# nsdumont/Semantic-Spiking-Neural-SLAM-2023

Measured on AMD Instinct MI355X. Metric: sim-sec/wall-sec, SSP-SLAM ssp_dim=1015 10k PI neurons, 1/2/4/8 MI355X, higher is better.
Workload: dtype f32; 1 GPU; PathIntegration 2-D ssp_dim=1015 pi_n_neurons=10000/VCO (508 VCOs, 5080000 LIF neurons), configs[1]; eval_points_per_vco=4000, parallelism=1 GPU, build_cache=miss

## Files before the change

semantic-spiking-neural-slam-2023_amd/csrc/ssn_block.hpp:

```cpp
#pragma once
#include <type_traits>
#include "ssn_launch.hpp"

namespace ssn {

__device__ inline float wave_sum_dpp(float v) {
  int x;
#define SSN_DPP_ADD(ctrl, rmask)                                                                             \
  x = __builtin_amdgcn_update_dpp(0, __builtin_bit_cast(int, v), ctrl, rmask, 0xF, false);                    \
  v += __builtin_bit_cast(float, x);
  SSN_DPP_ADD(0xB1, 0xF)
  SSN_DPP_ADD(0x4E, 0xF)
  SSN_DPP_ADD(0x141, 0xF)
  SSN_DPP_ADD(0x140, 0xF)
  SSN_DPP_ADD(0x142, 0xA)
  SSN_DPP_ADD(0x143, 0xC)
#undef SSN_DPP_ADD
  return v;
}
__device__ inline float row_sum_dpp(float v) {
  int x;
#define SSN_DPP_ADD(ctrl)                                                                                    \
  x = __builtin_amdgcn_update_dpp(0, __builtin_bit_cast(int, v), ctrl, 0xF, 0xF, false);                      \
  v += __builtin_bit_cast(float, x);
  SSN_DPP_ADD(0xB1) SSN_DPP_ADD(0x4E) SSN_DPP_ADD(0x141) SSN_DPP_ADD(0x140)
#undef SSN_DPP_ADD
  return v;
}
template <int N>
__device__ inline void wave_sum_dpp_n(float* v) {
#define SSN_DPP_STAGE(ctrl, rmask)                                                                            \
  _Pragma("unroll") for (int r = 0; r < N; ++r) {                                                              \
    const int x = __builtin_amdgcn_update_dpp(0, __builtin_bit_cast(int, v[r]), ctrl, rmask, 0xF, false);      \
    v[r] += __builtin_bit_cast(float, x);                                                                      \
  }
  SSN_DPP_STAGE(0xB1, 0xF) SSN_DPP_STAGE(0x4E, 0xF) SSN_DPP_STAGE(0x141, 0xF) SSN_DPP_STAGE(0x140, 0xF)
  SSN_DPP_STAGE(0x142, 0xA) SSN_DPP_STAGE(0x143, 0xC)
#undef SSN_DPP_STAGE
}
__device__ inline double wave_sum_dpp(double v) {
#pragma unroll
  for (int off = 32; off > 0; off >>= 1) v += __shfl_xor(v, off, 64);
  return v;
}
template <int N>
__device__ inline void wave_sum_dpp_n(double* v) {
#pragma unroll
  for (int r = 0; r < N; ++r) v[r] = wave_sum_dpp(v[r]);
}

typedef float f32x2 __attribute__((ext_vector_type(2)));
typedef unsigned int u32x2 __attribute__((ext_vector_type(2)));
__device__ inline f32x2 pk_clamp01(f32x2 x) {
  f32x2 r;
  asm("v_pk_mul_f32 %0, %1, 1.0 op_sel_hi:[1,0] clamp" : "=v"(r) : "v"(x));
  return r;
}
__device__ inline f32x2 pk_sub_clamp01(f32x2 x, f32x2 y) {
  f32x2 r;
  asm("v_pk_add_f32 %0, %1, %2 neg_lo:[0,1] neg_hi:[0,1] clamp" : "=v"(r) : "v"(x), "s"(y));
  return r;
}
__device__ inline f32x2 pk_mul_clamp01(f32x2 x, f32x2 y) {
  f32x2 r;
  asm("v_pk_mul_f32 %0, %1, %2 clamp" : "=v"(r) : "v"(x), "s"(y));
  return r;
}
__device__ inline f32x2 pk_fma_clamp01_vsv(f32x2 x, f32x2 y, f32x2 z) {
  f32x2 r;
  asm("v_pk_fma_f32 %0, %1, %2, %3 clamp" : "=v"(r) : "v"(x), "s"(y), "v"(z));
  return r;
}
__device__ inline f32x2 pk_fma_clamp01_trans_vvs(f32x2 x, f32x2 y, f32x2 z) {
  f32x2 r;
  asm("s_nop 0\n\tv_pk_fma_f32 %0, %1, %2, %3 clamp" : "=v"(r) : "v"(x), "v"(y), "s"(z));
  return r;
}

__device__ inline f32x2 pk_fma_clamp01_vs_negv(f32x2 x, f32x2 y, f32x2 z) {
  f32x2 r;
  asm("v_pk_fma_f32 %0, %1, %2, %3 neg_lo:[0,0,1] neg_hi:[0,0,1] clamp" : "=v"(r) : "v"(x), "s"(y), "v"(z));
  return r;
}

struct LifConstV3 { float na, ca, m1, c1, c2, c3, p0, p1, p2, ktau_ref, K; };
struct LifConstV3P { f32x2 na, ca, m1, c1, c2, c3, p0, p1, p2, ktau_ref; };

__device__ inline LifConstV3 lif_const_v3(double dt, double tau_rc, double tau_ref) {
  double K = 1.0;
  while (2.0 * K * tau_ref <= 1.0 && K < 1048576.0) K *= 2.0;
  while (K * tau_ref > 1.0) K *= 0.5;
  const double h = dt / tau_rc;
  const double x0 = h, x1 = 0.5 * h, x2 = 0.0669872981077807 * h;
  auto f = [](double x) { return -expm1(-x) / x; };
  const double f0 = f(x0), f1 = f(x1), f2 = f(x2);
  const double d01 = (f1 - f0) / (x1 - x0), d12 = (f2 - f1) / (x2 - x1), d012 = (d12 - d01) / (x2 - x0);
  const double q2 = d012, q1 = d01 - d012 * (x0 + x1), q0 = f0 - d01 * x0 + d012 * x0 * x1;
  LifConstV3 c;
  const float a = (float)(1.0 / (K * dt));
  float ca = a + 1.0f;
  if ((double)ca < (double)a + 1.0) ca = __builtin_bit_cast(float, __builtin_bit_cast(unsigned int, ca) + 1u);
  c.na = -a; c.ca = ca; c.m1 = (float)(1.0 + K * dt);
  c.c1 = (float)(q0 * h); c.c2 = (float)(q1 * h * h); c.c3 = (float)(q2 * h * h * h);
  {
    const double um = -expm1(-h);
    const double u0 = um * 0.9330127018922193, u1 = um * 0.5, u2 = um * 0.0669872981077807;
    auto phi = [](double u) { return log1p(-u) / u; };
    const double g0 = phi(u0), g1 = phi(u1), g2 = phi(u2);
    const double e01 = (g1 - g0) / (u1 - u0), e12 = (g2 - g1) / (u2 - u1), e012 = (e12 - e01) / (u2 - u0);
    const double r2 = e012, r1 = e01 - e012 * (u0 + u1), r0 = g0 - e01 * u0 + e012 * u0 * u1;
    c.p0 = (float)(K * tau_rc * r0); c.p1 = (float)(K * tau_rc * r1); c.p2 = (float)(K * tau_rc * r2);
  }
  c.ktau_ref = (float)(K * tau_ref); c.K = (float)K;
  return c;
}

__device__ inline f32x2 lif_state_dl(f32x2 w, f32x2 na, f32x2 ca) {
  return pk_fma_clamp01_vsv(w, (f32x2)(na), (f32x2)(ca));
}
__device__ inline f32x2 lif_state_p1(f32x2 dl, f32x2 c3, f32x2 c2) {
  f32x2 P;
  asm("v_pk_fma_f32 %0, %1, %2, %3" : "=v"(P) : "v"(dl), "v"((f32x2)(c3)), "s"((f32x2)(c2)));
  return P;
}
__device__ inline f32x2 lif_state_p2(f32x2 dl, f32x2 P, f32x2 c1) {
  asm("v_pk_fma_f32 %0, %1, %2, %3" : "=v"(P) : "v"(dl), "v"(P), "s"((f32x2)(c1)));
  return P;
}
__device__ inline void lif_state_part(f32x2 w, const LifConstV3P& c, f32x2& W0, f32x2& em) {
  W0 = pk_clamp01(w);
  const f32x2 dl = lif_state_dl(w, c.na, c.ca);
  const f32x2 P = lif_state_p2(dl, lif_state_p1(dl, c.c3, c.c2), c.c1);
  em = dl * P;
}
__device__ inline f32x2 lif_spike_test(f32x2 Jm1, f32x2 w, f32x2 W0, f32x2 em, const LifConstV3P& c, f32x2 big, f32x2& U, f32x2& nmt) {
  nmt = pk_sub_clamp01(w, (f32x2)(c.m1));
  U = __builtin_elementwise_fma(Jm1 + W0, em, -W0);
  return pk_mul_clamp01(U, big);
}
__device__ inline void lif_finish_spiking(f32x2 Jm1, f32x2& w, f32x2 U, f32x2 nmt, f32x2 spk, const LifConstV3P& c, f32x2 big) {
  f32x2 rc;
  rc.x = __builtin_amdgcn_rcpf(Jm1.x);
  rc.y = __builtin_amdgcn_rcpf(Jm1.y);
  const f32x2 u = U * rc;
  f32x2 P, nu;
  asm("v_pk_fma_f32 %0, %1, %2, %3" : "=v"(P) : "v"(u), "v"((f32x2)(c.p2)), "s"((f32x2)(c.p1)));
  asm("v_pk_fma_f32 %0, %1, %2, %3" : "=v"(P) : "v"(u), "v"(P), "s"((f32x2)(c.p0)));
  asm("v_pk_fma_f32 %0, %1, %2, %3 clamp" : "=v"(nu) : "v"(u), "v"(P), "s"((f32x2)(c.ktau_ref)));
  const f32x2 Wn = pk_fma_clamp01_vs_negv(spk, big, U);
  w = __builtin_elementwise_fma(spk, nu, Wn + nmt);
}
__device__ inline void lif_finish_silent(f32x2& w, f32x2 U, f32x2 nmt) {
  f32x2 Wn;
  asm("v_pk_mul_f32 %0, %1, -1.0 op_sel_hi:[1,0] clamp" : "=v"(Wn) : "v"(U));
  w = Wn + nmt;
}
__device__ inline f32x2 lif_input_part(f32x2 Jm1, f32x2& w, f32x2 W0, f32x2 em, const LifConstV3P& c, f32x2 big) {
  const f32x2 nmt = pk_sub_clamp01(w, (f32x2)(c.m1));
  const f32x2 U = __builtin_elementwise_fma(Jm1 + W0, em, -W0);
  const f32x2 spk = pk_mul_clamp01(U, big);
  f32x2 rc;
  rc.x = __builtin_amdgcn_rcpf(Jm1.x);
  rc.y = __builtin_amdgcn_rcpf(Jm1.y);
  f32x2 Wn, u, P, nu;
  asm("v_pk_fma_f32 %0, %2, %3, %4 neg_lo:[0,0,1] neg_hi:[0,0,1] clamp\n\t"
      "v_pk_mul_f32 %1, %4, %5"
      : "=&v"(Wn), "=v"(u)
      : "v"(spk), "s"(big), "v"(U), "v"(rc));
  asm("v_pk_fma_f32 %0, %1, %2, %3" : "=v"(P) : "v"(u), "v"((f32x2)(c.p2)), "s"((f32x2)(c.p1)));
  asm("v_pk_fma_f32 %0, %1, %2, %3" : "=v"(P) : "v"(u), "v"(P), "s"((f32x2)(c.p0)));
  asm("v_pk_fma_f32 %0, %1, %2, %3 clamp" : "=v"(nu) : "v"(u), "v"(P), "s"((f32x2)(c.ktau_ref)));
  w = __builtin_elementwise_fma(spk, nu, Wn + nmt);
  return spk;
}
__device__ inline float lif_word_in(float s, float K) { return __builtin_fmaf(-s, s < 0.0f ? K : 1.0f, 1.0f); }
__device__ inline float lif_word_out(float w, float K) { return (1.0f - w) * (w > 1.0f ? 1.0f / K : 1.0f); }

__device__ inline float bits_f(unsigned int x) { return __builtin_bit_cast(float, x); }
__device__ inline unsigned int f_bits(float x) { return __builtin_bit_cast(unsigned int, x); }

#ifdef SSN_BLOCK_STAMPS
__device__ unsigned long long g_block_stamps[9];
inline hipError_t read_block_stamps(unsigned long long* out, int reset) {
  hipError_t e = hipMemcpyFromSymbol(out, HIP_SYMBOL(g_block_stamps), sizeof(unsigned long long) * 9);
  if (e == hipSuccess && reset) {
    const unsigned long long z[9] = {0, 0, 0, 0, 0, 0, 0, 0, 0};
    e = hipMemcpyToSymbol(HIP_SYMBOL(g_block_stamps), z, sizeof z);
  }
  return e;
}
#define SSN_BSTAMP(var)                                                                          \
  do {                                                                                           \
    __builtin_amdgcn_sched_barrier(0);                                                           \
    asm volatile("s_memtime %0\n\ts_waitcnt lgkmcnt(0)" : "=s"(var) :: "memory");                \
    __builtin_amdgcn_sched_barrier(0);                                                           \
  } while (0)
#define SSN_BSTAMP_ADD(i, a, b) bst[i] += (b) - (a)
#else
#define SSN_BSTAMP(var) do {} while (0)
#define SSN_BSTAMP_ADD(i, a, b) do {} while (0)
#endif

#ifndef SSN_BLOCK_SKIP
#define SSN_BLOCK_SKIP 0
#endif
#ifndef SSN_BLOCK_PIPE
#define SSN_BLOCK_PIPE 1
#endif
#ifndef SSN_BLOCK_HOIST_A
#define SSN_BLOCK_HOIST_A 2
#endif
#ifndef SSN_BLOCK_HOIST_B
#define SSN_BLOCK_HOIST_B 4
#endif
#ifndef SSN_BLOCK_HOIST_C
#define SSN_BLOCK_HOIST_C 2
#endif
struct BlockHoist { int a, b, c; };
constexpr BlockHoist block_hoist(bool pipe, int tpb, int ng) {
  if (!pipe || SSN_BLOCK_SKIP != 0) return {0, 0, 0};
  const int room = tpb <= 512 && ng >= 10 ? ng : 0;
  const int c = SSN_BLOCK_HOIST_C >= 2 && room >= 2 ? 2 : 0;
  int b = SSN_BLOCK_HOIST_B < room - c ? SSN_BLOCK_HOIST_B : room - c;
  int a_ = SSN_BLOCK_HOIST_A < room - c - b ? SSN_BLOCK_HOIST_A : room - c - b;
  return {a_, b, c};
}

template <typename T, int DIN, int DOUT, int NPT, int TPB, int LDSW, int SPLIT = 0, int TAP = 0>
__global__ __launch_bounds__(TPB) void k_ens_block(BlockArgs<T> a) {
  static_assert(!(SPLIT && TAP), "the split kernel has no tapped form");
  constexpr bool ENC_LDS = LDSW == DIN;
  static_assert(LDSW == 0 || LDSW == DIN, "LDSW");
  extern __shared__ __align__(16) unsigned char ssn_block_dyn[];
  T* const e_lds = reinterpret_cast<T*>(ssn_block_dyn);
  constexpr bool F32 = sizeof(T) == 4;
  constexpr int PK = F32 ? 2 : 1;
  constexpr int NG = NPT / PK;
  static_assert(NPT % PK == 0, "f32 variants handle neuron pairs");
  constexpr bool PIPE = F32 && NG >= 5 && SSN_BLOCK_PIPE != 0;
  constexpr BlockHoist HO = block_hoist(PIPE, TPB, NG);
  constexpr int HC = HO.c, HA = HO.a, HB = HO.b, HT = HC + HA + HB;
  using G = typename std::conditional<F32, f32x2, T>::type;
  constexpr int DP = DOUT <= 4 ? 4 : 8;
  static_assert(!SPLIT || (sizeof(T) == 4 && DOUT <= 4), "split ensembles: f32, at most four decoded rows");
  const int P = SPLIT ? a.P : 1;
  const int k = P > 1 ? (int)blockIdx.x / P : (int)blockIdx.x;
  const int member = P > 1 ? (int)blockIdx.x - k * P : 0;
  const int noff = member * a.n_member;
  const int n_loc = P > 1 ? max(0, min(a.n_member, a.n_pad - noff)) : a.n_pad;
  const int tid = threadIdx.x;
  const int nthr = NG == 1 ? (int)blockDim.x : TPB;
  const int lane = tid & 63, wave = tid >> 6;
  const size_t row = (size_t)a.n_pad;
  const T* __restrict__ enc = a.enc + (size_t)k * DIN * row + noff;
  const T* __restrict__ bias = a.bias + (size_t)k * row + noff;
  T* __restrict__ Sp = a.S + (size_t)k * row + noff;
  const NeuronParams<T> np = a.np;
  const LifMath<T> lm(np);
  const int* tcol = nullptr;
  if constexpr (TAP != 0) {
    const int tslot = a.tap_slot[k];
    if (tslot >= 0) tcol = a.tap_col + (size_t)tslot * row;
  }
  auto uni = [](float v) { return bits_f(__builtin_amdgcn_readfirstlane(f_bits(v))); };
  const LifConstV3 lc0 = lif_const_v3((double)np.dt, (double)np.tau_rc, (double)np.tau_ref);
  auto uni2 = [&](float v) { const float u = uni(v); return (f32x2){u, u}; };
  const LifConstV3P lc = {uni2(lc0.na), uni2(lc0.ca), uni2(lc0.m1), uni2(lc0.c1), uni2(lc0.c2), uni2(lc0.c3), uni2(lc0.p0), uni2(lc0.p1),
                          uni2(lc0.p2), uni2(lc0.ktau_ref)};
  const float lcK = uni(lc0.K);
  const f32x2 big = {0x1p100f, 0x1p100f};

  G e[ENC_LDS ? 1 : NG][DIN], b[NG], s[NG], dc[NG][DOUT];
  constexpr int cap = (NG == 1 ? 1024 : TPB) * NPT;
  int lrow[LDSW > 0 ? LDSW : 1];
#pragma unroll
  for (int d = 0; d < (LDSW > 0 ? LDSW : 1); ++d) {
    lrow[d] = d * cap + tid * PK;
    asm volatile("" : "+v"(lrow[d]));
  }
  auto lds_group = [&](int d, int g) -> const G* {
    return reinterpret_cast<const G*>(e_lds + lrow[d] + g * nthr * PK);
  };
#pragma unroll
  for (int g = 0; g < NG; ++g) {
    const int i0 = (g * nthr + tid) * PK;
    const bool in = i0 < n_loc;
    const int ii = in ? i0 : 0;
    const T msk = in ? T(1) : T(0);
    auto ld = [&](const T* p) -> G { if constexpr (F32) return *reinterpret_cast<const f32x2*>(p) * msk; else return *p * msk; };
#pragma unroll
    for (int d = 0; d < DIN; ++d) {
      const G ev = ld(enc + d * row + ii);
      if constexpr (ENC_LDS) *reinterpret_cast<G*>(e_lds + d * cap + i0) = ev; else e[g][d] = ev;
    }
    b[g] = ld(bias + ii);
    s[g] = ld(Sp + ii);
    if constexpr (F32) {
      b[g] = b[g] - 1.0f;
      s[g] = (f32x2){lif_word_in(s[g].x, lcK), lif_word_in(s[g].y, lcK)};
    }
    if (a.dec_neuron_major) {
      const T* dp = a.dec + ((size_t)k * row + noff + ii) * DP;
#pragma unroll
      for (int r = 0; r < DOUT; ++r) {
        if constexpr (F32) dc[g][r] = (f32x2){dp[r], dp[DP + r]} * msk; else dc[g][r] = dp[r] * msk;
      }
    } else {
      const T* dp = a.dec + (size_t)k * DOUT * row + noff + ii;
#pragma unroll
      for (int r = 0; r < DOUT; ++r) dc[g][r] = ld(dp + r * row);
    }
  }

  constexpr int CH = 32;
  constexpr int XP = 4;
  constexpr int RW = DOUT <= 4 ? 64 : 128;
  __shared__ __align__(16) T red[2][RW];
  __shared__ __align__(16) T xs[CH][XP];
  __shared__ T os[CH][DOUT];
  __shared__ int s_dst[DOUT];
  __shared__ int s_out[DOUT];
  for (int i = tid; i < 2 * RW; i += nthr) (&red[0][0])[i] = T(0);
  if (tid < DOUT) { s_dst[tid] = a.didx[(long long)k * DOUT + tid]; s_out[tid] = a.rowout[(long long)k * DOUT + tid] ? 1 : 0; }
  const T* __restrict__ xbase = a.xrows + (size_t)a.row0 * a.n_sig + a.x_off + (long long)k * DIN;

  T fs[F32 ? 1 : DOUT], la[F32 ? 1 : DOUT], lb[F32 ? 1 : DOUT], tot[F32 ? 1 : DOUT];
  float F0 = 0.0f, F1 = 0.0f, la0 = 0.0f, lb0 = 0.0f, la1 = 0.0f, lb1 = 0.0f, v0 = 0.0f, v1 = 0.0f;
  T xa[DIN];
  int xr[DIN];
#pragma unroll
  for (int d = 0; d < DIN; ++d) {
    xr[d] = a.xrow[(long long)k * DIN + d];
    xa[d] = xr[d] >= 0 ? a.xalpha[(long long)k * DIN + d] : T(0);
  }
  if constexpr (F32) {
    const int r0 = lane >> 4;
    if (r0 < DOUT) {
      const long long i = (long long)k * DOUT + r0;
      const int st = a.lp_state[i];
      if (st >= 0) { F0 = a.sig[st]; la0 = a.lp_a[i]; lb0 = a.lp_b[i]; }
    }
    if (DOUT > 4) {
      const long long i = (long long)k * DOUT + 4;
      const int st = a.lp_state[i];
      if (st >= 0) { F1 = a.sig[st]; la1 = a.lp_a[i]; lb1 = a.lp_b[i]; }
    }
  } else {
#pragma unroll
    for (int r = 0; r < DOUT; ++r) {
      const long long i = (long long)k * DOUT + r;
      const int st = a.lp_state[i];
      fs[r] = st >= 0 ? a.sig[st] : T(0);
      la[r] = st >= 0 ? a.lp_a[i] : T(0);
      lb[r] = st >= 0 ? a.lp_b[i] : T(0);
      tot[r] = T(0);
    }
  }
  int wslot = -1;
  if constexpr (F32) {
    if constexpr (DOUT >= 4) {
      const int rv = (lane >> 4) == 1 ? 2 : ((lane >> 4) == 2 ? 1 : (lane >> 4));
      if ((lane & 15) == 0) wslot = rv * 16 + wave;
      if (DOUT == 5 && lane == 63) wslot = 64 + wave;
    }
  }

  constexpr int ILE = F32 ? (SSN_BLOCK_IL < NG ? SSN_BLOCK_IL : NG) : 1;
  G en[ILE][LDSW > 0 ? LDSW : 1];
  if constexpr (ENC_LDS) {
#pragma unroll
    for (int u = 0; u < ILE; ++u)
#pragma unroll
      for (int d = 0; d < LDSW; ++d) en[u][d] = *lds_group(d, u);
  }
#ifdef SSN_BLOCK_STAMPS
  unsigned long long bst[6] = {0, 0, 0, 0, 0, 0}, bt0 = 0, bt1 = 0, bt2 = 0, bt3 = 0, bt4 = 0, bt5 = 0, bt6 = 0, bm0 = 0, br0 = 0;
  asm volatile("s_memtime %0\n\ts_memrealtime %1\n\ts_waitcnt lgkmcnt(0)" : "=s"(bm0), "=s"(br0) :: "memory");
#endif
  unsigned int n_slots = 0, n_silent = 0;
  T x[DIN];
  int xl[DIN];
#pragma unroll
  for (int d = 0; d < DIN; ++d) xl[d] = __builtin_amdgcn_readfirstlane((xr[d] & 3) << 4);
  auto assemble_x = [&](const float4 xv) {
    const float xin[4] = {xv.x, xv.y, xv.z, xv.w};
    float f1 = 0.0f;
    if constexpr (DOUT > 4) f1 = bits_f(__builtin_amdgcn_readlane(f_bits(F1), 0));
#pragma unroll
    for (int d = 0; d < DIN; ++d) {
      const float f0 = bits_f(__builtin_amdgcn_readlane(f_bits(F0), xl[d]));
      float st = f0;
      if constexpr (DOUT > 4) st = xr[d] >= 4 ? f1 : f0;
      x[d] = __builtin_fmaf(xa[d], st, xin[d]);
    }
  };
  f32x2 W0h[HT > 0 ? HT : 1], emh[HT > 0 ? HT : 1];
  if constexpr (HT > 0) {
#pragma unroll
    for (int g = 0; g < HT; ++g) lif_state_part(s[g], lc, W0h[g], emh[g]);
  }
  for (int j0 = 0; j0 < a.B; j0 += CH) {
    const int cn = min(CH, a.B - j0);
    __syncthreads();
    if (j0 > 0 && member == 0) {
      for (int i = tid; i < CH * DOUT; i += nthr) {
        const int jj = i / DOUT, r = i - jj * DOUT;
        if (s_out[r]) a.bsig[(size_t)(a.row0 + j0 - CH + jj) * a.n_sig + s_dst[r]] = os[jj][r];
      }
    }
    for (int i = tid; i < cn * DIN; i += nthr) {
      const int jj = i / DIN, d = i - jj * DIN;
      xs[jj][d] = xbase[(size_t)(j0 + jj) * a.n_sig + d];
    }
    __syncthreads();
    if constexpr (PIPE) {
      assemble_x(*(const float4*)xs[0]);
    }

    for (int jj = 0; jj < cn; ++jj) {
      SSN_BSTAMP(bt0);
      if constexpr (SPLIT != 0) {
        if (P > 1 && wave == 0 && (lane & 15) == 0) {
          unsigned int* const rst = a.xslots + (size_t)k * 64 + (size_t)((j0 + jj + 1) % 3) * ((size_t)a.K * 64) + member * 4 + (lane >> 4);
          const unsigned int sent = BLOCK_XCHG_SENTINEL;
          asm volatile("global_store_dword %0, %1, off sc0 sc1" :: "v"(rst), "v"(sent) : "memory");
        }
      }
      if constexpr (PIPE) {
      } else if constexpr (F32) {
        assemble_x(*(const float4*)xs[jj]);
      } else {
        T xin[XP];
        *(double2*)xin = *(const double2*)xs[jj]; *(double2*)(xin + 2) = *(const double2*)(xs[jj] + 2);
#pragma unroll
        for (int d = 0; d < DIN; ++d) {
          T st = T(0);
#pragma unroll
          for (int r = 0; r < DOUT; ++r) st = xr[d] == r ? fs[r] : st;
          x[d] = xr[d] >= 0 ? xin[d] + xa[d] * st : xin[d];
        }
      }
      SSN_BSTAMP(bt1);
      G accg[DOUT];
#pragma unroll
      for (int r = 0; r < DOUT; ++r) accg[r] = G(0);
      constexpr int IL = ILE;
#pragma unroll
      for (int g0 = 0; g0 < NG; g0 += IL) {
        G J[IL], spk[IL];
#pragma unroll
        for (int u = 0; u < IL; ++u) {
          const int g = g0 + u < NG ? g0 + u : NG - 1;
          J[u] = b[g];
#pragma unroll
          for (int d = 0; d < DIN; ++d) {
            if constexpr (ENC_LDS) J[u] += en[u][d] * x[d];
            else J[u] += e[g][d] * x[d];
          }
        }
        if constexpr (ENC_LDS) {
#pragma unroll
          for (int u = 0; u < IL; ++u) {
            if (g0 + u >= NG) continue;
            asm volatile("" : "+v"(J[u]));
            const int gn = g0 + IL + u < NG ? g0 + IL + u : (g0 + IL + u) % IL;
#pragma unroll
            for (int d = 0; d < LDSW; ++d) en[u][d] = *lds_group(d, gn);
          }
        }
        bool at_rest = false;
        if constexpr (F32 && SSN_BLOCK_SKIP == 2) {
          ++n_slots;
          f32x2 r2 = {0.0f, 0.0f};
#pragma unroll
          for (int u = 0; u < IL; ++u) {
            if (g0 + u >= NG) continue;
            f32x2 pj;
            asm("v_pk_add_f32 %0, %1, 1.0 op_sel_hi:[1,0] clamp" : "=v"(pj) : "v"(J[u]));
            const f32x2 q = s[g0 + u] - 1.0f;
            r2 += __builtin_elementwise_fma(q, q, pj);
          }
          at_rest = __builtin_amdgcn_ballot_w64(__builtin_bit_cast(unsigned long long, r2) != 0ull) == 0ull;
          if (at_rest) ++n_silent;
        }
        if constexpr (F32 && SSN_BLOCK_SKIP == 1) {
          ++n_slots;
          f32x2 Uu[IL], nm[IL];
          f32x2 any2 = {0.0f, 0.0f};
#pragma unroll
          for (int u = 0; u < IL; ++u) {
            const int g = g0 + u < NG ? g0 + u : NG - 1;
            f32x2 W0, em;
            lif_state_part(s[g], lc, W0, em);
            spk[u] = lif_spike_test(J[u], s[g], W0, em, lc, big, Uu[u], nm[u]);
            if (g0 + u < NG) any2 += spk[u];
          }
          if (__builtin_amdgcn_ballot_w64(any2.x + any2.y != 0.0f) != 0ull) {
#pragma unroll
            for (int u = 0; u < IL; ++u)
              if (g0 + u < NG) lif_finish_spiking(J[u], s[g0 + u], Uu[u], nm[u], spk[u], lc, big);
#pragma unroll
            for (int u = 0; u < IL; ++u) {
              if (g0 + u >= NG) continue;
#pragma unroll
              for (int r = 0; r < DOUT; ++r) accg[r] = __builtin_elementwise_fma(spk[u], dc[g0 + u][r], accg[r]);
            }
          } else {
#pragma unroll
            for (int u = 0; u < IL; ++u)
              if (g0 + u < NG) lif_finish_silent(s[g0 + u], Uu[u], nm[u]);
            ++n_silent;
          }
        }
        if (!at_rest) {
#pragma unroll
        for (int u = 0; u < IL; ++u) {
          const int g = g0 + u;
          if (g >= NG) continue;
          if constexpr (F32 && SSN_BLOCK_SKIP == 1) {
          } else if constexpr (F32) {
            f32x2 W0, em;
            if (g < HT) { W0 = W0h[g < HT ? g : 0]; em = emh[g < HT ? g : 0]; }
            else lif_state_part(s[g], lc, W0, em);
            spk[u] = lif_input_part(J[u], s[g], W0, em, lc, big);
          } else {
            const T sw = s[g];
            T V = sw < T(0) ? T(0) : sw;
            T R = (sw < T(0) ? -sw : T(0)) - np.dt;
            T delta = np.dt - R;
            delta = delta < T(0) ? T(0) : (delta > np.dt ? np.dt : delta);
            V = V - (J[u] - V) * lm.decay(delta);
            spk[u] = T(0);
            if (V > T(1)) {
              const T t_spike = np.dt + np.tau_rc * lm.spike_time_term(V, J[u]);
              R = np.tau_ref + t_spike;
              V = T(0);
              spk[u] = T(1);
            } else if (V < T(0)) {
              V = T(0);
            }
            s[g] = R > np.dt ? -R : V;
          }
        }
#pragma unroll
        for (int u = 0; u < IL; ++u) {
          const int g = g0 + u;
          if (g >= NG) continue;
          if constexpr (F32) asm volatile("" : "+v"(s[g]));
          if constexpr (TAP != 0) {
            if (tcol) {
              const int i0 = (g * nthr + tid) * PK;
              T* const trow = a.bsig + (size_t)(a.row0 + j0 + jj) * a.n_sig;
              if (i0 < n_loc) {
                if constexpr (F32) {
                  const int2 d = *reinterpret_cast<const int2*>(tcol + i0);
                  const f32x2 val = spk[u] * a.tap_amp;
                  if (d.x >= 0) trow[d.x] = val.x;
                  if (d.y >= 0) trow[d.y] = val.y;
                } else {
                  const int d = tcol[i0];
                  if (d >= 0) trow[d] = spk[u] * a.tap_amp;
                }
              }
            }
          }
          if constexpr (F32 && SSN_BLOCK_SKIP == 1) continue;
#pragma unroll
          for (int r = 0; r < DOUT; ++r) {
            if constexpr (F32) accg[r] = __builtin_elementwise_fma(spk[u], dc[g][r], accg[r]);
            else accg[r] = fma(spk[u], dc[g][r], accg[r]);
          }
        }
        }
#ifndef SSN_BLOCK_NO_SCHED_BARRIER
        if constexpr (F32) __builtin_amdgcn_sched_barrier(0);
#endif
      }
      const int par = jj & 1;
      SSN_BSTAMP(bt2);
      if constexpr (F32) {
        float4 xnx = {0.0f, 0.0f, 0.0f, 0.0f};
        if constexpr (PIPE) xnx = *(const float4*)xs[jj + 1 < cn ? jj + 1 : jj];
        (void)xnx;
        float acc[DOUT];
#pragma unroll
        for (int r = 0; r < DOUT; ++r) acc[r] = accg[r].x + accg[r].y;
        if constexpr (DOUT >= 4) {
          const auto p01 = __builtin_amdgcn_permlane32_swap(f_bits(acc[0]), f_bits(acc[1]), false, false);
          const auto p23 = __builtin_amdgcn_permlane32_swap(f_bits(acc[2]), f_bits(acc[3]), false, false);
          const float s01 = bits_f(p01[0]) + bits_f(p01[1]);
          const float s23 = bits_f(p23[0]) + bits_f(p23[1]);
          const auto q = __builtin_amdgcn_permlane16_swap(f_bits(s01), f_bits(s23), false, false);
          float t4 = bits_f(q[0]) + bits_f(q[1]);
          t4 = row_sum_dpp(t4);
          if constexpr (DOUT == 5) {
            const float w4 = wave_sum_dpp(acc[4]);
            if (wslot >= 0) red[par][wslot] = lane == 63 ? w4 : t4;
          } else {
            if (wslot >= 0) red[par][wslot] = t4;
          }
        } else {
          wave_sum_dpp_n<DOUT>(acc);
          if (lane == 63) {
#pragma unroll
            for (int r = 0; r < DOUT; ++r) red[par][r * 16 + wave] = acc[r];
          }
        }
        if constexpr (HA > 0) {
          __builtin_amdgcn_sched_barrier(0);
#pragma unroll
          for (int g = HC; g < HC + HA; ++g) lif_state_part(s[g], lc, W0h[g], emh[g]);
          __builtin_amdgcn_sched_barrier(0);
        }
        SSN_BSTAMP(bt3);
        __syncthreads();
        SSN_BSTAMP(bt4);
        if constexpr (PIPE) {
          const float rv = red[par][lane];
          float rv1 = 0.0f;
          if constexpr (DOUT > 4) rv1 = red[par][64 + lane];
          if constexpr (HB > 0) {
            __builtin_amdgcn_sched_barrier(0);
#pragma unroll
            for (int g = HC + HA; g < HT; ++g) lif_state_part(s[g], lc, W0h[g], emh[g]);
            __builtin_amdgcn_sched_barrier(0);
          }
          if constexpr (HC == 2) {
            f32x2 dl0, dl1, P0, P1;
            v0 = rv;
            asm volatile(
                "v_pk_fma_f32 %1, %7, %9, %10 clamp\n\t"
                "v_pk_fma_f32 %2, %8, %9, %10 clamp\n\t"
                "v_add_f32_dpp %0, %0, %0 quad_perm:[1,0,3,2] row_mask:0xf bank_mask:0xf bound_ctrl:1\n\t"
                "v_pk_fma_f32 %3, %1, %11, %12\n\t"
                "v_pk_fma_f32 %4, %2, %11, %12\n\t"
                "v_add_f32_dpp %0, %0, %0 quad_perm:[2,3,0,1] row_mask:0xf bank_mask:0xf bound_ctrl:1\n\t"
                "v_pk_fma_f32 %3, %1, %3, %13\n\t"
                "v_pk_fma_f32 %4, %2, %4, %13\n\t"
                "v_add_f32_dpp %0, %0, %0 row_half_mirror row_mask:0xf bank_mask:0xf bound_ctrl:1\n\t"
                "v_pk_mul_f32 %5, %1, %3\n\t"
                "v_pk_mul_f32 %6, %2, %4\n\t"
                "v_add_f32_dpp %0, %0, %0 row_mirror row_mask:0xf bank_mask:0xf bound_ctrl:1"
                : "+v"(v0), "=&v"(dl0), "=&v"(dl1), "=&v"(P0), "=&v"(P1), "=&v"(emh[0]), "=&v"(emh[1])
                : "v"(s[0]), "v"(s[1]), "s"(lc.na), "v"(lc.ca), "v"(lc.c3), "s"(lc.c2), "s"(lc.c1));
          } else {
            v0 = row_sum_dpp(rv);
          }
          if constexpr (DOUT > 4) v1 = rv1;
        } else {
          v0 = row_sum_dpp(red[par][lane]);
        }
        SSN_BSTAMP(bt5);
        if constexpr (SPLIT != 0) {
          if (P > 1) {
            const int tq = j0 + jj;
            unsigned int* const xb = a.xslots + (size_t)k * 64;
            const size_t bstride = (size_t)a.K * 64;
            if (wave == 0 && (lane & 15) == 0) {
              unsigned int* const pub = xb + (size_t)(tq % 3) * bstride + member * 4 + (lane >> 4);
              const unsigned int val = f_bits(v0);
              asm volatile("s_waitcnt vmcnt(0)\n\tglobal_store_dword %0, %1, off sc0 sc1" :: "v"(pub), "v"(val) : "memory");
            }
            const unsigned int* const src = xb + (size_t)(tq % 3) * bstride + (lane & 15) * 4 + (lane >> 4);
            const bool mine = (lane & 15) < P;
            unsigned int got = 0, spins = 0;
            while (true) {
              if (mine) asm volatile("global_load_dword %0, %1, off sc0 sc1\n\ts_waitcnt vmcnt(0)" : "=v"(got) : "v"(src) : "memory");
              if (!__any(mine && got == BLOCK_XCHG_SENTINEL)) break;
              if (++spins > (1u << 20)) { if (lane == 0) *a.xerr = 1; break; }
            }
            v0 = row_sum_dpp(mine ? bits_f(got) : 0.0f);
          }
        }
        F0 = __builtin_fmaf(la0, F0, lb0 * v0);
        if constexpr (HC > 0) {
          __builtin_amdgcn_sched_barrier(0);
#pragma unroll
          for (int g = 0; g < HC; ++g) W0h[g] = pk_clamp01(s[g]);
          __builtin_amdgcn_sched_barrier(0);
        }
        if constexpr (DOUT > 4) {
          if constexpr (PIPE) v1 = row_sum_dpp(v1); else v1 = row_sum_dpp(red[par][64 + lane]);
          F1 = __builtin_fmaf(la1, F1, lb1 * v1);
        }
        if constexpr (PIPE) assemble_x(xnx);
        if (wave == 0 && member == 0) {
          if ((lane & 15) == 0 && (lane >> 4) < DOUT) os[jj][lane >> 4] = v0;
          if (DOUT > 4 && lane == 0) os[jj][4] = v1;
        }
        SSN_BSTAMP(bt6);
        SSN_BSTAMP_ADD(0, bt0, bt1); SSN_BSTAMP_ADD(1, bt1, bt2); SSN_BSTAMP_ADD(2, bt2, bt3); SSN_BSTAMP_ADD(3, bt3, bt4);
        SSN_BSTAMP_ADD(4, bt4, bt6); SSN_BSTAMP_ADD(5, bt4, bt5);
      } else {
        T acc[DOUT];
#pragma unroll
        for (int r = 0; r < DOUT; ++r) acc[r] = accg[r];
        wave_sum_dpp_n<DOUT>(acc);
        if (lane == 63) {
#pragma unroll
          for (int r = 0; r < DOUT; ++r) red[par][r * 16 + wave] = acc[r];
        }
        __syncthreads();
#pragma unroll
        for (int r = 0; r < DOUT; ++r) {
          T t = T(0);
#pragma unroll
          for (int w = 0; w < 16; ++w) t += red[par][r * 16 + w];
          tot[r] = t;
        }
#pragma unroll
        for (int r = 0; r < DOUT; ++r) fs[r] = la[r] * fs[r] + lb[r] * tot[r];
        if (tid < DOUT) {
          T v = T(0);
#pragma unroll
          for (int r = 0; r < DOUT; ++r) v = tid == r ? tot[r] : v;
          os[jj][tid] = v;
        }
      }
    }
  }
#ifdef SSN_BLOCK_STAMPS
  if constexpr (F32) {
    unsigned long long bm1, br1;
    asm volatile("s_memtime %0\n\ts_memrealtime %1\n\ts_waitcnt lgkmcnt(0)" : "=s"(bm1), "=s"(br1) :: "memory");
    if (lane == 0) {
      for (int i = 0; i < 5; ++i) atomicAdd(&g_block_stamps[i], bst[i]);
      atomicAdd(&g_block_stamps[8], bst[5]);
      atomicAdd(&g_block_stamps[5], (unsigned long long)a.B);
      if (k == 0 && wave == 0) { atomicAdd(&g_block_stamps[6], bm1 - bm0); atomicAdd(&g_block_stamps[7], br1 - br0); }
    }
  }
#endif
  if constexpr (F32 && SSN_BLOCK_SKIP != 0) {
    if (lane == 0 && a.slot_stats) {
      atomicAdd(a.slot_stats, (unsigned long long)n_slots);
      atomicAdd(a.slot_stats + 1, (unsigned long long)n_silent);
    }
  }
  __syncthreads();
  if (member == 0) {
    const int j0 = (a.B - 1) / CH * CH, cn = a.B - j0;
    for (int i = tid; i < cn * DOUT; i += nthr) {
      const int jj = i / DOUT, r = i - jj * DOUT;
      if (s_out[r]) a.bsig[(size_t)(a.row0 + j0 + jj) * a.n_sig + s_dst[r]] = os[jj][r];
    }
  }

  int tid2 = tid;
  asm volatile("" : "+v"(tid2));
#pragma unroll
  for (int g = 0; g < NG; ++g) {
    const int i0 = (g * nthr + tid2) * PK;
    if constexpr (F32) s[g] = (f32x2){lif_word_out(s[g].x, lcK), lif_word_out(s[g].y, lcK)};
    if (i0 < n_loc) *reinterpret_cast<G*>(Sp + i0) = s[g];
  }
  if constexpr (TAP != 0) {
    if (tcol && a.B > 0) {
      const T* const lrow = a.bsig + (size_t)(a.row0 + a.B - 1) * a.n_sig;
#pragma unroll
      for (int g = 0; g < NG; ++g) {
        const int i0 = (g * nthr + tid2) * PK;
        if (i0 >= n_loc) continue;
#pragma unroll
        for (int c = 0; c < PK; ++c) {
          const int d = tcol[i0 + c];
          if (d >= 0) a.sig_w[d] = lrow[d];
        }
      }
    }
  }
  if (a.B > 0 && member == 0) {
    if constexpr (F32) {
      if (wave == 0 && (lane & 15) == 0 && (lane >> 4) < DOUT) {
        const int r = lane >> 4;
        a.sig_w[s_dst[r]] = v0;
        const int st = a.lp_state[(long long)k * DOUT + r];
        if (st >= 0) a.sig_w[st] = F0;
      }
      if (DOUT > 4 && tid == 0) {
        a.sig_w[s_dst[4]] = v1;
        const int st = a.lp_state[(long long)k * DOUT + 4];
        if (st >= 0) a.sig_w[st] = F1;
      }
    } else if (tid < DOUT) {
      T v = T(0), f = T(0);
#pragma unroll
      for (int r = 0; r < DOUT; ++r) { v = tid == r ? tot[r] : v; f = tid == r ? fs[r] : f; }
      a.sig_w[s_dst[tid]] = v;
      const int st = a.lp_state[(long long)k * DOUT + tid];
      if (st >= 0) a.sig_w[st] = f;
    }
  }
}

constexpr int BLOCK_LDS_BYTES = 160 * 1024, BLOCK_STATIC_LDS = 2560;

template <typename T, int DIN, int DOUT, int NPT, int TPB, int LDSW, int SPLIT, int TAP = 0>
static hipError_t launch_block_variant_s(hipStream_t s, const BlockArgs<T>& a) {
  const int lds = LDSW * a.threads * NPT * (int)sizeof(T);
  static std::atomic<uint64_t> configured{0};
  if (LDSW > 0) {
    hipError_t e = set_max_dynamic_lds_once(reinterpret_cast<const void*>(&k_ens_block<T, DIN, DOUT, NPT, TPB, LDSW, SPLIT, TAP>),
                                            BLOCK_LDS_BYTES - BLOCK_STATIC_LDS, configured);
    if (e != hipSuccess) return e;
  }
  hipLaunchKernelGGL((k_ens_block<T, DIN, DOUT, NPT, TPB, LDSW, SPLIT, TAP>), dim3((unsigned)(a.K * (SPLIT ? a.P : 1))), dim3((unsigned)a.threads), lds, s, a);
  return hipGetLastError();
}
template <typename T, int DIN, int DOUT, int NPT, int TPB, int LDSW>
static hipError_t launch_block_variant(hipStream_t s, const BlockArgs<T>& a) {
  if (a.P > 1) {
    if constexpr (sizeof(T) == 4 && DOUT <= 4) return launch_block_variant_s<T, DIN, DOUT, NPT, TPB, LDSW, 1>(s, a);
    else return hipErrorInvalidValue;
  }
  if (a.tap_slot) {
    if constexpr (SSN_BLOCK_SKIP == 0) return launch_block_variant_s<T, DIN, DOUT, NPT, TPB, LDSW, 0, 1>(s, a);
    else return hipErrorInvalidValue;
  }
  return launch_block_variant_s<T, DIN, DOUT, NPT, TPB, LDSW, 0>(s, a);
}

struct BlockVariant { int tpb, npt, ldsw; };
template <typename T> struct BlockVariants;
template <> struct BlockVariants<float> {
  static constexpr int N = 7;
  static constexpr BlockVariant v[N] = {{1024, 2, 0}, {1024, 4, 0}, {512, 6, 0}, {1024, 6, 0}, {512, 10, 0}, {512, 20, 3}, {768, 14, 3}};
};
template <> struct BlockVariants<double> {
  static constexpr int N = 3;
  static constexpr BlockVariant v[N] = {{1024, 1, 0}, {1024, 2, 0}, {1024, 4, 0}};
};

template <typename T, int DIN, int DOUT>
static hipError_t launch_block_npt(hipStream_t s, const BlockArgs<T>& a) {
  const int key = (a.tpb * 100 + a.npt) * 8 + a.enc_lds;
  switch (key) {
#define SSN_CASE(TPB, N, L) case (TPB * 100 + N) * 8 + L: return launch_block_variant<T, DIN, DOUT, N, TPB, L>(s, a);
    SSN_CASE(1024, 2, 0) SSN_CASE(1024, 4, 0)
#undef SSN_CASE
#define SSN_CASE(TPB, N, L) case (TPB * 100 + N) * 8 + L: if constexpr (sizeof(T) == 8) return launch_block_variant<T, DIN, DOUT, N, TPB, L>(s, a); else return hipErrorInvalidValue;
    SSN_CASE(1024, 1, 0)
#undef SSN_CASE
#define SSN_CASE(TPB, N, L) case (TPB * 100 + N) * 8 + L: if constexpr (sizeof(T) == 4) return launch_block_variant<T, DIN, DOUT, N, TPB, L>(s, a); else return hipErrorInvalidValue;
    SSN_CASE(1024, 6, 0) SSN_CASE(512, 6, 0) SSN_CASE(512, 10, 0) SSN_CASE(512, 20, 3) SSN_CASE(768, 14, 3)
#undef SSN_CASE
    default: return hipErrorInvalidValue;
  }
}

template <typename T>
bool ens_block_supported(int din, int dout, int n, const int want[3], int* threads, int* tpb, int* npt, int* enc_lds) {
  if (!(din == 3 && dout >= 3 && dout <= 5)) return false;
  const int want_tpb = want[0], want_npt = want[1], want_lds = want[2];
  const int pk = sizeof(T) == 4 ? 2 : 1;
  for (int i = 0; i < BlockVariants<T>::N; ++i) {
    const BlockVariant v = BlockVariants<T>::v[i];
    if (want_tpb && (v.tpb != want_tpb || v.npt != want_npt || v.ldsw != want_lds)) continue;
    int th = v.tpb;
    if (v.npt == pk && n < th * pk) th = std::max(64, ((n + pk - 1) / pk + 63) / 64 * 64);
    if ((int64_t)th * v.npt < n) continue;
    if ((int64_t)v.ldsw * th * v.npt * (int64_t)sizeof(T) > BLOCK_LDS_BYTES - BLOCK_STATIC_LDS) continue;
    *threads = th; *tpb = v.tpb; *npt = v.npt; *enc_lds = v.ldsw;
    return true;
  }
  return false;
}

template <typename T>
hipError_t launch_ens_block(hipStream_t s, const BlockArgs<T>& a) {
  if (a.din == 3 && a.dout == 5) return launch_block_npt<T, 3, 5>(s, a);
  if (a.din == 3 && a.dout == 4) return launch_block_npt<T, 3, 4>(s, a);
  if (a.din == 3 && a.dout == 3) return launch_block_npt<T, 3, 3>(s, a);
  return hipErrorInvalidValue;
}

}
```

Before: 359.1 sim-sec/wall-sec.

## Batch prologue loads, size row chunks from free LDS, prefill first chunk

Restructures the block kernel prologue so encoder, bias, state and decoder loads for several neuron groups are issued together before masking and conversion, and the per-ensemble scalar words are loaded branch-free. This exposes more memory-level parallelism at kernel start. The staged input/output row buffers move from fixed static LDS (32 rows) into dynamic LDS, with the chunk size picked from the remaining LDS budget. This cuts the number of chunk-boundary syncs and bsig write-back rounds, and the first chunk is prefetched early with wider unrolled loads. The trade-offs are higher register pressure from the batched loads and a larger LDS footprint per block, which may lower occupancy. The change also adds optional timing stamps.

Measured after the change: 354.3 sim-sec/wall-sec. 0.987x the previous value.

```diff
diff --git a/semantic-spiking-neural-slam-2023_amd/csrc/ssn_block.hpp b/semantic-spiking-neural-slam-2023_amd/csrc/ssn_block.hpp
--- a/semantic-spiking-neural-slam-2023_amd/csrc/ssn_block.hpp
+++ b/semantic-spiking-neural-slam-2023_amd/csrc/ssn_block.hpp
@@ -180,11 +180,12 @@
 __device__ inline unsigned int f_bits(float x) { return __builtin_bit_cast(unsigned int, x); }
 
 #ifdef SSN_BLOCK_STAMPS
-__device__ unsigned long long g_block_stamps[9];
+constexpr int BLOCK_NSTAMPS = 16;
+__device__ unsigned long long g_block_stamps[BLOCK_NSTAMPS];
 inline hipError_t read_block_stamps(unsigned long long* out, int reset) {
-  hipError_t e = hipMemcpyFromSymbol(out, HIP_SYMBOL(g_block_stamps), sizeof(unsigned long long) * 9);
+  hipError_t e = hipMemcpyFromSymbol(out, HIP_SYMBOL(g_block_stamps), sizeof(unsigned long long) * BLOCK_NSTAMPS);
   if (e == hipSuccess && reset) {
-    const unsigned long long z[9] = {0, 0, 0, 0, 0, 0, 0, 0, 0};
+    const unsigned long long z[BLOCK_NSTAMPS] = {};
     e = hipMemcpyToSymbol(HIP_SYMBOL(g_block_stamps), z, sizeof z);
   }
   return e;
@@ -226,6 +227,27 @@
   return {a_, b, c};
 }
 
+#ifndef SSN_BLOCK_CHUNK
+#define SSN_BLOCK_CHUNK 0
+#endif
+#ifndef SSN_BLOCK_BATCH_LOADS
+#define SSN_BLOCK_BATCH_LOADS 1
+#endif
+constexpr int block_batch_groups(int tpb, int ng) {
+  if (SSN_BLOCK_BATCH_LOADS == 0) return 1;
+  const int nb = SSN_BLOCK_BATCH_LOADS > 1 ? SSN_BLOCK_BATCH_LOADS : (tpb > 512 ? 4 : ng);
+  return nb < ng ? nb : ng;
+}
+constexpr int BLOCK_LDS_BYTES = 160 * 1024;
+constexpr int block_static_lds(int tsize, int dout) { return 2 * (dout <= 4 ? 64 : 128) * tsize + 2 * dout * 4; }
+constexpr int block_io_lds(int tsize, int dout, int ch) { return ch * (4 + dout) * tsize; }
+constexpr int block_chunk(int tsize, int dout, int enc_bytes) {
+  if (SSN_BLOCK_CHUNK > 0) return SSN_BLOCK_CHUNK;
+  int ch = 1024;
+  while (ch > 32 && enc_bytes + block_io_lds(tsize, dout, ch) + block_static_lds(tsize, dout) > BLOCK_LDS_BYTES) ch /= 2;
+  return ch;
+}
+
 template <typename T, int DIN, int DOUT, int NPT, int TPB, int LDSW, int SPLIT = 0, int TAP = 0>
 __global__ __launch_bounds__(TPB) void k_ens_block(BlockArgs<T> a) {
   static_assert(!(SPLIT && TAP), "the split kernel has no tapped form");
@@ -236,6 +258,10 @@
   constexpr bool F32 = sizeof(T) == 4;
   constexpr int PK = F32 ? 2 : 1;
   constexpr int NG = NPT / PK;
+#ifdef SSN_BLOCK_STAMPS
+  unsigned long long be0 = 0;
+  asm volatile("s_memtime %0\n\ts_waitcnt lgkmcnt(0)" : "=s"(be0) :: "memory");
+#endif
   static_assert(NPT % PK == 0, "f32 variants handle neuron pairs");
   constexpr bool PIPE = F32 && NG >= 5 && SSN_BLOCK_PIPE != 0;
   constexpr BlockHoist HO = block_hoist(PIPE, TPB, NG);
@@ -281,81 +307,150 @@
   auto lds_group = [&](int d, int g) -> const G* {
     return reinterpret_cast<const G*>(e_lds + lrow[d] + g * nthr * PK);
   };
-#pragma unroll
-  for (int g = 0; g < NG; ++g) {
+  auto ld = [&](const T* p) -> G { if constexpr (F32) return *reinterpret_cast<const f32x2*>(p); else return *p; };
+  auto group_load = [&](int g, G (&ev)[DIN]) {
     const int i0 = (g * nthr + tid) * PK;
-    const bool in = i0 < n_loc;
-    const int ii = in ? i0 : 0;
-    const T msk = in ? T(1) : T(0);
-    auto ld = [&](const T* p) -> G { if constexpr (F32) return *reinterpret_cast<const f32x2*>(p) * msk; else return *p * msk; };
-#pragma unroll
-    for (int d = 0; d < DIN; ++d) {
-      const G ev = ld(enc + d * row + ii);
-      if constexpr (ENC_LDS) *reinterpret_cast<G*>(e_lds + d * cap + i0) = ev; else e[g][d] = ev;
-    }
+    const int ii = i0 < n_loc ? i0 : 0;
+#pragma unroll
+    for (int d = 0; d < DIN; ++d) ev[d] = ld(enc + d * row + ii);
     b[g] = ld(bias + ii);
     s[g] = ld(Sp + ii);
+  };
+  auto group_load_dec = [&](int g, auto nm) {
+    const int i0 = (g * nthr + tid) * PK;
+    const int ii = i0 < n_loc ? i0 : 0;
+    if (nm) {
+      const T* dp = a.dec + ((size_t)k * row + noff + ii) * DP;
+#pragma unroll
+      for (int r = 0; r < DOUT; ++r) {
+        if constexpr (F32) dc[g][r] = (f32x2){dp[r], dp[DP + r]}; else dc[g][r] = dp[r];
+      }
+    } else {
+      const T* dp = a.dec + (size_t)k * DOUT * row + noff + ii;
+#pragma unroll
+      for (int r = 0; r < DOUT; ++r) dc[g][r] = ld(dp + r * row);
+    }
+  };
+  auto group_finish = [&](int g, const G (&ev)[DIN]) {
+    const int i0 = (g * nthr + tid) * PK;
+    const T msk = i0 < n_loc ? T(1) : T(0);
+#pragma unroll
+    for (int d = 0; d < DIN; ++d) {
+      if constexpr (ENC_LDS) *reinterpret_cast<G*>(e_lds + d * cap + i0) = ev[d] * msk; else e[g][d] = ev[d] * msk;
+    }
+    b[g] = b[g] * msk;
+    s[g] = s[g] * msk;
     if constexpr (F32) {
       b[g] = b[g] - 1.0f;
       s[g] = (f32x2){lif_word_in(s[g].x, lcK), lif_word_in(s[g].y, lcK)};
     }
-    if (a.dec_neuron_major) {
-      const T* dp = a.dec + ((size_t)k * row + noff + ii) * DP;
-#pragma unroll
-      for (int r = 0; r < DOUT; ++r) {
-        if constexpr (F32) dc[g][r] = (f32x2){dp[r], dp[DP + r]} * msk; else dc[g][r] = dp[r] * msk;
-      }
-    } else {
-      const T* dp = a.dec + (size_t)k * DOUT * row + noff + ii;
-#pragma unroll
-      for (int r = 0; r < DOUT; ++r) dc[g][r] = ld(dp + r * row);
-    }
-  }
-
-  constexpr int CH = 32;
+#pragma unroll
+    for (int r = 0; r < DOUT; ++r) dc[g][r] = dc[g][r] * msk;
+  };
+
+  constexpr int ENC_BYTES = LDSW * cap * (int)sizeof(T);
+  constexpr int CH = block_chunk((int)sizeof(T), DOUT, ENC_BYTES);
   constexpr int XP = 4;
   constexpr int RW = DOUT <= 4 ? 64 : 128;
+  static_assert(CH >= 1 && ENC_BYTES % 16 == 0 && (CH * XP * (int)sizeof(T)) % 16 == 0, "staged rows: 16-byte aligned");
+  static_assert(ENC_BYTES + block_io_lds((int)sizeof(T), DOUT, CH) + block_static_lds((int)sizeof(T), DOUT) <= BLOCK_LDS_BYTES, "LDS budget");
   __shared__ __align__(16) T red[2][RW];
-  __shared__ __align__(16) T xs[CH][XP];
-  __shared__ T os[CH][DOUT];
   __shared__ int s_dst[DOUT];
   __shared__ int s_out[DOUT];
-  for (int i = tid; i < 2 * RW; i += nthr) (&red[0][0])[i] = T(0);
-  if (tid < DOUT) { s_dst[tid] = a.didx[(long long)k * DOUT + tid]; s_out[tid] = a.rowout[(long long)k * DOUT + tid] ? 1 : 0; }
+  static_assert(sizeof(red) + sizeof(s_dst) + sizeof(s_out) == block_static_lds((int)sizeof(T), DOUT), "block_static_lds");
+  T (*const xs)[XP] = reinterpret_cast<T (*)[XP]>(ssn_block_dyn + ENC_BYTES);
+  T (*const os)[DOUT] = reinterpret_cast<T (*)[DOUT]>(ssn_block_dyn + ENC_BYTES + CH * XP * (int)sizeof(T));
   const T* __restrict__ xbase = a.xrows + (size_t)a.row0 * a.n_sig + a.x_off + (long long)k * DIN;
+  auto rows_fill = [&](int j0, int cn, auto width) {
+    constexpr int U = decltype(width)::value;
+    for (int base = 0; base < cn * DIN; base += U * nthr) {
+      T xw[U];
+#pragma unroll
+      for (int u = 0; u < U; ++u) {
+        const int i = min(base + tid + u * nthr, cn * DIN - 1);
+        const int jj = i / DIN, d = i - jj * DIN;
+        xw[u] = xbase[(size_t)(j0 + jj) * a.n_sig + d];
+      }
+#pragma unroll
+      for (int u = 0; u < U; ++u) {
+        const int i = base + tid + u * nthr;
+        const int jj = i / DIN, d = i - jj * DIN;
+        if (i < cn * DIN) xs[jj][d] = xw[u];
+      }
+    }
+  };
+  constexpr bool ROWS_FIRST = SSN_BLOCK_BATCH_LOADS != 0;
+  if constexpr (ROWS_FIRST) {
+    if (a.B > 0) rows_fill(0, min(CH, a.B), std::integral_constant<int, 8>{});
+  }
 
   T fs[F32 ? 1 : DOUT], la[F32 ? 1 : DOUT], lb[F32 ? 1 : DOUT], tot[F32 ? 1 : DOUT];
   float F0 = 0.0f, F1 = 0.0f, la0 = 0.0f, lb0 = 0.0f, la1 = 0.0f, lb1 = 0.0f, v0 = 0.0f, v1 = 0.0f;
   T xa[DIN];
   int xr[DIN];
-#pragma unroll
-  for (int d = 0; d < DIN; ++d) {
-    xr[d] = a.xrow[(long long)k * DIN + d];
-    xa[d] = xr[d] >= 0 ? a.xalpha[(long long)k * DIN + d] : T(0);
-  }
-  if constexpr (F32) {
-    const int r0 = lane >> 4;
-    if (r0 < DOUT) {
-      const long long i = (long long)k * DOUT + r0;
-      const int st = a.lp_state[i];
-      if (st >= 0) { F0 = a.sig[st]; la0 = a.lp_a[i]; lb0 = a.lp_b[i]; }
-    }
-    if (DOUT > 4) {
-      const long long i = (long long)k * DOUT + 4;
-      const int st = a.lp_state[i];
-      if (st >= 0) { F1 = a.sig[st]; la1 = a.lp_a[i]; lb1 = a.lp_b[i]; }
-    }
-  } else {
-#pragma unroll
-    for (int r = 0; r < DOUT; ++r) {
-      const long long i = (long long)k * DOUT + r;
-      const int st = a.lp_state[i];
-      fs[r] = st >= 0 ? a.sig[st] : T(0);
-      la[r] = st >= 0 ? a.lp_a[i] : T(0);
-      lb[r] = st >= 0 ? a.lp_b[i] : T(0);
-      tot[r] = T(0);
-    }
-  }
+  int w_dst = 0, w_out = 0;
+  auto ensemble_words = [&]() {
+    const long long io = (long long)k * DOUT + min(tid, DOUT - 1);
+    w_dst = a.didx[io];
+    w_out = a.rowout[io] ? 1 : 0;
+#pragma unroll
+    for (int d = 0; d < DIN; ++d) {
+      xr[d] = a.xrow[(long long)k * DIN + d];
+      xa[d] = a.xalpha[(long long)k * DIN + d];
+    }
+    if constexpr (F32) {
+      const int r0 = lane >> 4;
+      {
+        const long long i = (long long)k * DOUT + min(r0, DOUT - 1);
+        const int st = a.lp_state[i];
+        la0 = a.lp_a[i]; lb0 = a.lp_b[i];
+        F0 = a.sig[max(st, 0)];
+        if (!(r0 < DOUT && st >= 0)) { F0 = 0.0f; la0 = 0.0f; lb0 = 0.0f; }
+      }
+      if constexpr (DOUT > 4) {
+        const long long i = (long long)k * DOUT + 4;
+        const int st = a.lp_state[i];
+        la1 = a.lp_a[i]; lb1 = a.lp_b[i];
+        F1 = a.sig[max(st, 0)];
+        if (st < 0) { F1 = 0.0f; la1 = 0.0f; lb1 = 0.0f; }
+      }
+    } else {
+#pragma unroll
+      for (int r = 0; r < DOUT; ++r) {
+        const long long i = (long long)k * DOUT + r;
+        const int st = a.lp_state[i];
+        fs[r] = a.sig[max(st, 0)]; la[r] = a.lp_a[i]; lb[r] = a.lp_b[i];
+        if (st < 0) { fs[r] = T(0); la[r] = T(0); lb[r] = T(0); }
+        tot[r] = T(0);
+      }
+    }
+  };
+  constexpr int NB = block_batch_groups(TPB, NG);
+#pragma unroll
+  for (int g0 = 0; g0 < NG; g0 += NB) {
+    G ev[NB][DIN];
+    if constexpr (NB > 1) {
+      if (a.dec_neuron_major) {
+#pragma unroll
+        for (int g = g0; g < g0 + NB && g < NG; ++g) group_load_dec(g, std::true_type{});
+      } else {
+#pragma unroll
+        for (int g = g0; g < g0 + NB && g < NG; ++g) group_load_dec(g, std::false_type{});
+      }
+#pragma unroll
+      for (int g = g0; g < g0 + NB && g < NG; ++g) group_load(g, ev[g - g0]);
+    } else {
+      group_load(g0, ev[0]);
+      group_load_dec(g0, a.dec_neuron_major != 0);
+    }
+#pragma unroll
+    for (int g = g0; g < g0 + NB && g < NG; ++g) group_finish(g, ev[g - g0]);
+  }
+  ensemble_words();
+#pragma unroll
+  for (int d = 0; d < DIN; ++d) xa[d] = xr[d] >= 0 ? xa[d] : T(0);
+  for (int i = tid; i < 2 * RW; i += nthr) (&red[0][0])[i] = T(0);
+  if (tid < DOUT) { s_dst[tid] = w_dst; s_out[tid] = w_out; }
   int wslot = -1;
   if constexpr (F32) {
     if constexpr (DOUT >= 4) {
@@ -375,6 +470,7 @@
   }
 #ifdef SSN_BLOCK_STAMPS
   unsigned long long bst[6] = {0, 0, 0, 0, 0, 0}, bt0 = 0, bt1 = 0, bt2 = 0, bt3 = 0, bt4 = 0, bt5 = 0, bt6 = 0, bm0 = 0, br0 = 0;
+  unsigned long long bb0 = 0, bb1 = 0, bpro = 0, bbnd = 0, nbnd = 0;
   asm volatile("s_memtime %0\n\ts_memrealtime %1\n\ts_waitcnt lgkmcnt(0)" : "=s"(bm0), "=s"(br0) :: "memory");
 #endif
   unsigned int n_slots = 0, n_silent = 0;
@@ -401,6 +497,9 @@
   }
   for (int j0 = 0; j0 < a.B; j0 += CH) {
     const int cn = min(CH, a.B - j0);
+#ifdef SSN_BLOCK_STAMPS
+    SSN_BSTAMP(bb0);
+#endif
     __syncthreads();
     if (j0 > 0 && member == 0) {
       for (int i = tid; i < CH * DOUT; i += nthr) {
@@ -408,14 +507,15 @@
         if (s_out[r]) a.bsig[(size_t)(a.row0 + j0 - CH + jj) * a.n_sig + s_dst[r]] = os[jj][r];
       }
     }
-    for (int i = tid; i < cn * DIN; i += nthr) {
-      const int jj = i / DIN, d = i - jj * DIN;
-      xs[jj][d] = xbase[(size_t)(j0 + jj) * a.n_sig + d];
-    }
+    if (j0 > 0 || !ROWS_FIRST) rows_fill(j0, cn, std::integral_constant<int, 1>{});
     __syncthreads();
     if constexpr (PIPE) {
       assemble_x(*(const float4*)xs[0]);
     }
+#ifdef SSN_BLOCK_STAMPS
+    SSN_BSTAMP(bb1);
+    if (j0 == 0) bpro = bb1 - be0; else { bbnd += bb1 - bb0; ++nbnd; }
+#endif
 
     for (int jj = 0; jj < cn; ++jj) {
       SSN_BSTAMP(bt0);
@@ -791,19 +891,33 @@
       if (st >= 0) a.sig_w[st] = f;
     }
   }
-}
-
-constexpr int BLOCK_LDS_BYTES = 160 * 1024, BLOCK_STATIC_LDS = 2560;
+#ifdef SSN_BLOCK_STAMPS
+  if constexpr (F32) {
+    unsigned long long be1;
+    asm volatile("s_waitcnt vmcnt(0)\n\ts_memtime %0\n\ts_waitcnt lgkmcnt(0)" : "=s"(be1) :: "memory");
+    if (wave == 0 && lane == 0 && a.B > 0) {
+      atomicAdd(&g_block_stamps[9], bpro);
+      atomicAdd(&g_block_stamps[10], bbnd);
+      atomicAdd(&g_block_stamps[11], nbnd);
+      atomicAdd(&g_block_stamps[12], be1 - bt6);
+      atomicAdd(&g_block_stamps[13], 1ull);
+      atomicAdd(&g_block_stamps[14], be1 - be0);
+      g_block_stamps[15] = (unsigned long long)a.B;
+    }
+  }
+#endif
+}
 
 template <typename T, int DIN, int DOUT, int NPT, int TPB, int LDSW, int SPLIT, int TAP = 0>
 static hipError_t launch_block_variant_s(hipStream_t s, const BlockArgs<T>& a) {
-  const int lds = LDSW * a.threads * NPT * (int)sizeof(T);
+  constexpr int enc_bytes = LDSW * TPB * NPT * (int)sizeof(T);
+  constexpr int lds = enc_bytes + block_io_lds((int)sizeof(T), DOUT, block_chunk((int)sizeof(T), DOUT, enc_bytes));
+  static_assert(lds + block_static_lds((int)sizeof(T), DOUT) <= BLOCK_LDS_BYTES, "LDS budget");
+  if (LDSW > 0 && a.threads != TPB) return hipErrorInvalidValue;
   static std::atomic<uint64_t> configured{0};
-  if (LDSW > 0) {
-    hipError_t e = set_max_dynamic_lds_once(reinterpret_cast<const void*>(&k_ens_block<T, DIN, DOUT, NPT, TPB, LDSW, SPLIT, TAP>),
-                                            BLOCK_LDS_BYTES - BLOCK_STATIC_LDS, configured);
-    if (e != hipSuccess) return e;
-  }
+  if (hipError_t e = set_max_dynamic_lds_once(reinterpret_cast<const void*>(&k_ens_block<T, DIN, DOUT, NPT, TPB, LDSW, SPLIT, TAP>), lds, configured);
+      e != hipSuccess)
+    return e;
   hipLaunchKernelGGL((k_ens_block<T, DIN, DOUT, NPT, TPB, LDSW, SPLIT, TAP>), dim3((unsigned)(a.K * (SPLIT ? a.P : 1))), dim3((unsigned)a.threads), lds, s, a);
   return hipGetLastError();
 }
@@ -859,7 +973,9 @@
     int th = v.tpb;
     if (v.npt == pk && n < th * pk) th = std::max(64, ((n + pk - 1) / pk + 63) / 64 * 64);
     if ((int64_t)th * v.npt < n) continue;
-    if ((int64_t)v.ldsw * th * v.npt * (int64_t)sizeof(T) > BLOCK_LDS_BYTES - BLOCK_STATIC_LDS) continue;
+    const int enc_bytes = v.ldsw * th * v.npt * (int)sizeof(T);
+    const int ch = block_chunk((int)sizeof(T), dout, enc_bytes);
+    if (enc_bytes + block_io_lds((int)sizeof(T), dout, ch) + block_static_lds((int)sizeof(T), dout) > BLOCK_LDS_BYTES) continue;
     *threads = th; *tpb = v.tpb; *npt = v.npt; *enc_lds = v.ldsw;
     return true;
   }
```
